# harrywaugh/UOB_Raytracer

Hardware: AMD Instinct MI355X
Metric: Mrays/sec (nominal = W*H*AA*(1+S)/t), Cornell Box 4096^2, 8xAA, 64 shadow rays (higher is better)
Workload: dtype f32; 1 GPU; headline: Cornell Box 4096x4096, 4x2 AA, 64 shadow rays, 2 spheres, <=10 bounces, 26 triangles; parallelism=1 GPU

## Files before the change

include/uob_rt.h:

```cpp
#ifndef UOB_RT_H
#define UOB_RT_H

#include <stddef.h>
#include <stdint.h>

#ifdef __cplusplus
extern "C" {
#endif

#define RT_ABI_VERSION 2
#define RT_MAX_SPHERES 4
#define RT_MAX_DEVICES 8

enum {
  RT_OK = 0,
  RT_E_INVALID = -1,
  RT_E_DEVICE = -2,
  RT_E_NOMEM = -3,
  RT_E_IO = -4,
  RT_E_UNSUPPORTED = -5
};

typedef struct rt_sphere {
  float center[3];
// ... 108 lines not shown
  float*   normal4;
  float*   albedo4;
  float*   direction4;
} rt_aov_buffers;

#define RT_AOV_ALL_SAMPLES (-1)
int rt_render_aov(rt_ctx* ctx, const float rot[12], const float cam[3], float focal, int32_t sample,
                  const rt_aov_buffers* host_out);
int rt_render_aov_device(rt_ctx* ctx, const float rot[12], const float cam[3], float focal, int32_t sample,
                         const rt_aov_buffers* device_out, void* hip_stream);
int rt_debug_aov_stats(rt_ctx* ctx, uint64_t out[8]);

int rt_debug_block_costs(rt_ctx* ctx, uint32_t* out, int32_t cap);

int rt_debug_world_masks(rt_ctx* ctx, uint64_t* out, int64_t cap, int32_t* grid, int32_t* words);

int rt_debug_tile_data(rt_ctx* ctx, int32_t* orig, float* tiles, int32_t cap_tiles);

int rt_register_output(rt_ctx* ctx, void* host, size_t bytes);
int rt_unregister_output(rt_ctx* ctx);

int rt_debug_wave_timeline(rt_ctx* ctx, uint64_t out[8]);

enum { RT_COPY_2D = 0,
       RT_COPY_PEER = 1,
       RT_COPY_LINEAR = 2    };
typedef struct rt_band_copy {
  int32_t op, reserved;
  uint64_t dst_offset, dst_pitch, src_offset, src_pitch, width_bytes, rows;
} rt_band_copy;
int rt_debug_band_copy_plan(int32_t num_devices, int32_t k, int32_t device_band_rows, int32_t width, int32_t height,
                            int32_t elem_bytes, int32_t dev_to_dev, int32_t peer_ok, int32_t same_device,
                            rt_band_copy* out, int32_t cap);

int rt_selftest_rcp(uint64_t out[64]);

int rt_selftest_normalize(uint64_t out[8], uint32_t b_stride);

void rt_destroy(rt_ctx* ctx);
const char* rt_last_error(void);
int rt_abi_version(void);

typedef struct rt_triangle {
  float v0[4], v1[4], v2[4], normal[4], color[4];
} rt_triangle;

// ... 14 lines not shown
```

uob_raytracer_amd/csrc/rt_api.hip:

```cpp
#include <cmath>
#include <cstdarg>
#include <cstdio>
#include <cstdlib>
#include <cstring>
#include <new>
#include <string>
#include <vector>

#include "rt_host.h"

namespace uobrt {

static thread_local std::string g_last_error;

void set_error(const char* fmt, ...) {
  char buf[1024];
  va_list ap;
  va_start(ap, fmt);
  vsnprintf(buf, sizeof buf, fmt, ap);
  va_end(ap);
  g_last_error = buf;
}

KeepError::KeepError() : text(g_last_error) {}
// ... 18 lines not shown
  if (!(c->light_spread >= 0.0f) || !(c->light_spread <= kMaxCoordinate)) { set_error("light_spread must be in [0, 2^16]"); return RT_E_INVALID; }
  if (validate_spheres(c->spheres, c->num_spheres) != RT_OK) return RT_E_INVALID;
  if ((double)c->width * c->height > 16777216.0) {
    set_error("width*height must not exceed 2^24 (the reference's FP32 pixel id)"); return RT_E_INVALID;
  }
  if (c->flags & 1) { set_error("flag bit 0 (the former RT_FLAG_FAST_MATH) is not defined in ABI %d", RT_ABI_VERSION); return RT_E_UNSUPPORTED; }
  if (c->num_devices < 0 || c->num_devices > RT_MAX_DEVICES || c->device_band_rows < 0) {
    set_error("num_devices must be in [0,%d] and device_band_rows >= 0", RT_MAX_DEVICES); return RT_E_INVALID;
  }
  if (c->num_devices > 1 && c->band_count != 1) {
    set_error("several devices in one context need the whole frame (band_count == 1)"); return RT_E_UNSUPPORTED;
  }
  return RT_OK;
}

static Tuning read_tuning(const rt_config& cfg) {
  Tuning t;
  if (const char* e = getenv("UOB_RT_JOB_TASKS")) t.job_tasks = atoi(e);
  if (const char* e = getenv("UOB_RT_HEAVY_FACTOR4")) { const int v = atoi(e); if (v >= 1 && v <= 4096) t.heavy_factor4 = v; }
  t.plain_order = (cfg.flags & RT_FLAG_PLAIN_ORDER) != 0 || getenv("UOB_RT_PLAIN_ORDER") != nullptr;
  t.full_grid = getenv("UOB_RT_FULL_GRID") != nullptr;
  t.no_specialise = getenv("UOB_RT_NO_SPECIALISE") != nullptr;
  if (const char* e = getenv("UOB_RT_HEAVY_DILATE")) t.heavy_dilate = atoi(e) != 0;
  if (const char* e = getenv("UOB_RT_L1_INFLATE")) { const float v = (float)atof(e); if (v >= 1.0f && v <= 64.0f) t.l1_inflate = v; }
  if (const char* e = getenv("UOB_RT_GRID_PER_CU")) { const int v = atoi(e); if (v >= 1 && v <= 8) t.grid_per_cu = v; }
  t.phase_profile = getenv("UOB_RT_PHASE_PROFILE") != nullptr;
  t.timeline = getenv("UOB_RT_TIMELINE") != nullptr;
  if (const char* e = getenv("UOB_RT_MASK_DEBUG")) t.mask_debug = atoi(e);
  if (const char* e = getenv("UOB_RT_TILE_ORDER")) t.tile_morton = !strcmp(e, "morton");
  return t;
}

extern "C" {

int rt_abi_version(void) { return RT_ABI_VERSION; }
const char* rt_last_error(void) { return g_last_error.c_str(); }

void rt_config_default(rt_config* cfg) {
  if (!cfg) return;
  memset(cfg, 0, sizeof *cfg);
  cfg->width = 1024; cfg->height = 1024;
  cfg->aa_x = 2; cfg->aa_y = 2;
  cfg->shadow_samples = 10; cfg->light_spread = 0.05f;
  cfg->max_bounces = 10;
  cfg->num_spheres = 2;
  const rt_sphere glass = {{0.3f, 0.1f, -0.5f}, 0.075f, {0.0f, 0.f, 0.f, -1.0f}};
// ... 75 lines not shown
  if (rc != RT_OK) return rc;
  if (n < 0 || (n > 0 && (!vertices4 || !normals4 || !colors4))) { set_error("scene arrays missing"); return RT_E_INVALID; }
  rc = validate_vertices(vertices4, n);
  if (rc != RT_OK) return rc;
  if (n > 4000000) { set_error("triangle list of %d exceeds the supported maximum of 4000000", n); return RT_E_UNSUPPORTED; }
  DeviceGuard guard;
  if (cfg->num_devices > 1) return init_parent(cfg, vertices4, normals4, colors4, n, out_ctx);
  int ndev = 0;
  HIP_TRY(hipGetDeviceCount(&ndev));
  if (ndev < 1) { set_error("no HIP device present"); return RT_E_DEVICE; }
  rt_ctx* c = new (std::nothrow) rt_ctx();
  if (!c) { set_error("out of host memory"); return RT_E_NOMEM; }
  c->cfg = *cfg;
  c->tune = read_tuning(*cfg);
  if (cfg->num_devices == 1) c->device = cfg->devices[0];
  else if (cfg->device >= 0) c->device = cfg->device;
  else hipGetDevice(&c->device);
  auto fail = [&](int code) { rt_destroy(c); return code; };
  if (hipSetDevice(c->device) != hipSuccess) { set_error("hipSetDevice(%d) failed", c->device); return fail(RT_E_DEVICE); }
  c->owned_rows = rt_config_owned_rows(cfg);
  if (hipDeviceGetAttribute(&c->cus, hipDeviceAttributeMultiprocessorCount, c->device) != hipSuccess || c->cus < 1) c->cus = 256;
  const size_t px = (size_t)(c->owned_rows > 0 ? c->owned_rows : 1) * cfg->width;
  if (hipMalloc(&c->d_argb, px * 4) != hipSuccess || hipMalloc(&c->d_counters, sizeof(rt_work)) != hipSuccess ||
      hipMalloc(&c->d_jobctr, (2 * kJobHeads + 2) * kJobHeadStride * sizeof(unsigned int)) != hipSuccess ||
      hipMalloc(&c->d_spheres, RT_MAX_SPHERES * sizeof(DevSphere)) != hipSuccess) {
    set_error("hipMalloc failed: %s", hipGetErrorString(hipGetLastError())); return fail(RT_E_NOMEM);
  }
  {
    const int aa = cfg->aa_x * cfg->aa_y;
    const int pt = (aa >= 1 && aa <= 64) ? 64 / aa : 16;
    const size_t jobs_max = (size_t)((cfg->width + pt - 1) / pt) * (size_t)(c->owned_rows > 0 ? c->owned_rows : 1);
    c->heavy_cap = (int)(jobs_max / 3 > 64 ? jobs_max / 3 : 64);
    c->heavy_jobs_max = jobs_max;
  }
  if (hipStreamCreate(&c->stream) != hipSuccess || hipEventCreate(&c->ev0) != hipSuccess || hipEventCreate(&c->ev1) != hipSuccess) {
    set_error("stream/event creation failed"); return fail(RT_E_DEVICE);
  }
  rc = upload_spheres(c);
  if (rc != RT_OK) return fail(rc);
  rc = scene_first(c, vertices4, normals4, colors4, n);
  if (rc != RT_OK) return fail(rc);
  *out_ctx = c;
  return RT_OK;
}

}

void uobrt::fill_params(const rt_ctx* c, const float rot[12], const float cam[3], const float light[3], float focal,
                        FrameParams* P) {
// ... 116 lines not shown
    if (!(fabsf(rot[k]) <= 4.0f)) { set_error("rotation matrix entries must be finite and <= 4"); return RT_E_INVALID; }
  if (c->owned_rows == 0) return RT_OK;
  FrameParams P;
  fill_params(c, rot, cam, light, focal, &P);
  P.out_argb = d_argb; P.out_rgb = d_rgb; P.counters = nullptr;
  P.out_global = out_global ? 1 : 0;
  HIP_TRY(hipSetDevice(c->device));
  if (c->timed && stream != c->last_stream) HIP_TRY(hipStreamWaitEvent(stream, c->ev1, 0));
  HIP_TRY(wait_aov(c, stream));
  HIP_TRY(wait_scene(c, stream));
  HIP_TRY(hipEventRecord(c->ev0, stream));
  const bool wave_paths = !(c->cfg.flags & RT_FLAG_GENERIC_KERNEL);
  if (wave_paths && wave_kernel_supports(P) && (P.aa_x * P.aa_y <= 64 || !(c->cfg.flags & RT_FLAG_NO_CULL))) {
    if (c->d_heavy_flags && P.job_tasks >= 4) {
      const int prev = c->heavy_phase, cur = prev ^ 1;
      unsigned int* const st[2] = {c->d_jobctr, c->d_jobctr + (2 * kJobHeads + 1) * kJobHeadStride};
      P.heavy_prev = c->d_heavy[prev]; P.heavy_prev_state = st[prev];
      P.heavy_new = c->d_heavy[cur]; P.heavy_new_state = st[cur];
      P.heavy_flags = c->d_heavy_flags + (size_t)prev * c->heavy_jobs_max; P.heavy_flags_new = c->d_heavy_flags + (size_t)cur * c->heavy_jobs_max;
      P.heavy_gen = ++c->heavy_gen;
      P.heavy_factor4 = c->tune.heavy_factor4;
      P.heavy_cap = P.njobs / 3 < c->heavy_cap ? P.njobs / 3 : c->heavy_cap;
      P.heavy_dilate = c->tune.heavy_dilate ? 1 : 0;
      c->heavy_phase = cur;
    }
    c->timeline_valid = false;
    if (c->tune.timeline) {
      const size_t waves = (size_t)P.wave_blocks * 4;
      if (!c->d_timeline) {
        if (hipMalloc(&c->d_timeline, waves * 3 * sizeof(uint64_t)) != hipSuccess) { set_error("hipMalloc failed (timeline)"); return RT_E_NOMEM; }
        c->timeline_waves = waves;
      }
      if (c->timeline_waves >= waves) {
        HIP_TRY(hipMemsetAsync(c->d_timeline, 0, c->timeline_waves * 3 * sizeof(uint64_t), stream));
        P.counters = reinterpret_cast<unsigned long long*>(c->d_timeline);
        c->timeline_valid = true;
      }
    }
    launch_wave(P, !(c->cfg.flags & RT_FLAG_NO_CULL), false, stream);
  } else if (wave_paths && !(c->cfg.flags & RT_FLAG_NO_CULL) && mesh_kernel_supports(P)) {
    use_tiled_scene(c, &P);
    if (c->d_mesh_cost) {
      P.mesh_order = c->mesh_order_valid ? c->d_mesh_order : nullptr;
      P.mesh_cost = c->d_mesh_cost; P.mesh_order_out = c->d_mesh_order;
      P.mesh_queue_len = c->d_mesh_order + 4 * (size_t)((c->cfg.width + 15) / 16) * (size_t)((c->owned_rows + 15) / 16);
      c->mesh_order_valid = true;
    }
    launch_stage_records(P, stream);
    launch_mesh(P, false, false, stream, c->aux_stream, c->ev_fork, c->ev_join);
  } else {
    launch_generic(P, false, stream);
  }
  HIP_TRY(hipGetLastError());
  HIP_TRY(hipEventRecord(c->ev1, stream));
  c->timed = true;
  c->last_stream = stream;
  return RT_OK;
// ... 267 lines not shown
  if (c->timed) HIP_TRY(hipStreamWaitEvent(c->stream, c->ev1, 0));
  HIP_TRY(wait_aov(c, c->stream));
  HIP_TRY(wait_scene(c, c->stream));
  HIP_TRY(hipMemsetAsync(c->d_counters, 0, sizeof(rt_work), c->stream));
  if (mesh) { use_tiled_scene(c, &P); launch_stage_records(P, c->stream); launch_mesh(P, true, c->tune.phase_profile, c->stream, nullptr, nullptr, nullptr); }
  else if (c->tune.phase_profile) launch_wave_prof(P, c->stream);
  else launch_wave(P, !(c->cfg.flags & RT_FLAG_NO_CULL), true, c->stream);
  HIP_TRY(hipGetLastError());
  HIP_TRY(hipMemcpyAsync(out, c->d_counters, sizeof(rt_work), hipMemcpyDeviceToHost, c->stream));
  HIP_TRY(hipStreamSynchronize(c->stream));
  return RT_OK;
}

int rt_debug_wave_timeline(rt_ctx* c, uint64_t out[8]) {
  if (!c || !out) { set_error("NULL argument"); return RT_E_INVALID; }
  c = lead_ctx(c);
  if (!c->tune.timeline || !c->timeline_valid) {
    set_error("rt_debug_wave_timeline: needs UOB_RT_TIMELINE=1 at rt_init and a frame rendered by the wave kernel");
    return RT_E_UNSUPPORTED;
  }
  DeviceGuard guard;
  HIP_TRY(hipSetDevice(c->device));
  if (c->timed) HIP_TRY(hipEventSynchronize(c->ev1));
  std::vector<uint64_t> rec(c->timeline_waves * 3);
  HIP_TRY(hipMemcpy(rec.data(), c->d_timeline, rec.size() * sizeof(uint64_t), hipMemcpyDeviceToHost));
  for (int q = 0; q < 8; ++q) out[q] = 0;
  out[1] = ~0ull;
  for (size_t w = 0; w < c->timeline_waves; ++w) {
    const uint64_t t0 = rec[3 * w], t1 = rec[3 * w + 1], jobs = rec[3 * w + 2] & 0xffffffffull;
    if (t1 == 0) continue;
    out[7] = rec[3 * w + 2] >> 32;
    out[0] += 1; out[3] += t0; out[4] += t1; out[5] += jobs;
    if (t0 < out[1]) out[1] = t0;
    if (t1 > out[2]) out[2] = t1;
    if (jobs > out[6]) out[6] = jobs;
  }
  return RT_OK;
}

int rt_debug_trace_rays(rt_ctx* c, int32_t what, const float* rays6, const float* radius_sq, int64_t nray,
                        int32_t* out_tri, float* out10) {
  if (!c || !rays6 || !out_tri || nray < 0) { set_error("NULL argument"); return RT_E_INVALID; }
  if (what != RT_TRACE_IN_SHADOW && what != RT_TRACE_CLOSEST_HIT) { set_error("rt_debug_trace_rays: unknown mode %d", what); return RT_E_INVALID; }
  if (what == RT_TRACE_IN_SHADOW && !radius_sq) { set_error("rt_debug_trace_rays: radius_sq missing"); return RT_E_INVALID; }
  if (what == RT_TRACE_CLOSEST_HIT && !out10) { set_error("rt_debug_trace_rays: out10 missing"); return RT_E_INVALID; }
  c = lead_ctx(c);
  if (nray == 0) return RT_OK;
  DeviceGuard guard;
  HIP_TRY(hipSetDevice(c->device));
  const float zero3[3] = {0.f, 0.f, 0.f};
  FrameParams P;
  scene_params(c, zero3, false, &P);
  float *d_rays = nullptr, *d_r2 = nullptr, *d_out = nullptr;
  int* d_tri = nullptr;
  int rc = RT_OK;
  if (hipMalloc(&d_rays, (size_t)nray * 24) != hipSuccess || hipMalloc(&d_tri, (size_t)nray * 4) != hipSuccess ||
      (radius_sq && hipMalloc(&d_r2, (size_t)nray * 4) != hipSuccess) || (out10 && hipMalloc(&d_out, (size_t)nray * 40) != hipSuccess)) {
    set_error("hipMalloc failed: %s", hipGetErrorString(hipGetLastError())); rc = RT_E_NOMEM;
// ... 128 lines not shown
```

uob_raytracer_amd/csrc/rt_device.h:

```cpp
#pragma once
#include <hip/hip_runtime.h>
#include <stdint.h>

#include "../../include/uob_rt.h"

namespace uobrt {

constexpr int kJobHeads = 31;
constexpr int kJobHeadStride = 32;
constexpr int kHeavyStateWords = 8;
constexpr float kMaxCoordinate = 65536.0f;
constexpr int kRecordsPerTriangle = 8;

struct DevSphere {
  float cx, cy, cz, r2;
  float col[4];
};

struct FrameParams {
  float rot[12];
  float cam[3];
  float focal;
  float light[3];
  float spread;
  int32_t W, H, aa_x, aa_y;
  int32_t S;
  int32_t bounces;
  int32_t nsph;
  int32_t n;
  int32_t band_rows, band_index, band_count, owned_rows;
  float sy;
  float half_wx, half_hy;
  float w_f;
// ... 13 lines not shown
  const float4* colors;
  uint32_t* out_argb;
  float4* out_rgb;
  int32_t out_global;
  int32_t wave_blocks;
  unsigned long long* counters;
  unsigned int* job_counter;
  int32_t njobs, nseg;
  int32_t aa_magic;
  int32_t aax_magic;
  int32_t job_tasks;
  int32_t no_specialise;
  const unsigned int* heavy_prev;
  const unsigned int* heavy_prev_state;
  unsigned int* heavy_new;
  unsigned int* heavy_new_state;
  const unsigned int* heavy_flags;
  unsigned int* heavy_flags_new;
  uint32_t heavy_gen;
  int32_t heavy_factor4;
  int32_t heavy_cap;
  float l1_inflate;
  int32_t heavy_dilate;
  float4* records;
  const unsigned int* mesh_order;
  unsigned int* mesh_cost;
  unsigned int* mesh_order_out;
  unsigned int* mesh_queue_len;
  int32_t mesh_blocks;
  const int* orig;
  const float4* tile_box;
  unsigned long long* screen_masks;
  unsigned long long* world_masks;
  unsigned int* world_occ;
  int32_t mask_debug;
  int32_t nwords, scx, scy, grid_g;
  float grid_lo[3], grid_cell, grid_inv;
};

struct AovPlanes {
  int* prim;
  float* depth;
  float4 *position, *normal, *albedo, *direction;
};

__device__ inline uint32_t div_magic(uint32_t n, uint32_t magic) { return magic ? __umulhi(n, magic) : n; }
// ... 13 lines not shown
```

uob_raytracer_amd/csrc/rt_host.h:

```cpp
#pragma once
#include <hip/hip_runtime.h>

#include <string>
#include <vector>

#include "rt_device.h"

#define HIP_TRY(expr)                                                                   \
  do {                                                                                  \
    hipError_t e_ = (expr);                                                             \
    if (e_ != hipSuccess) {                                                             \
      uobrt::set_error("%s failed: %s (%s:%d)", #expr, hipGetErrorString(e_), __FILE__, __LINE__); \
      return RT_E_DEVICE;                                                               \
    }                                                                                   \
  } while (0)

namespace uobrt {

void set_error(const char* fmt, ...);

struct KeepError {
  std::string text;
  KeepError();
  ~KeepError();
// ... 37 lines not shown
                     int* d_prim, float4* d_records, unsigned long long* stats, int cus, hipStream_t stream);
int aov_stats_words();
void launch_aov(const FrameParams& P, bool tiled, const AovPlanes& A, int sample, unsigned long long* stats, int cus, hipStream_t stream);
void vertex_box(const float* vertices4, int n, float lo[3], float hi[3]);
std::vector<int> tiled_order(const float* v4, int n, bool morton);
std::vector<float> tile_data_host(const float* v4, const int* orig, int n);

inline uint32_t div_magic_for(int d) { return d > 1 ? (uint32_t)((0x100000000ull + (uint64_t)d - 1) / (uint64_t)d) : 0u; }

inline int blocks_per_cu(const void* kernel, int threads) {
  int per_cu = 0;
  if (hipOccupancyMaxActiveBlocksPerMultiprocessor(&per_cu, kernel, threads, 0) != hipSuccess || per_cu < 1) per_cu = 2;
  return per_cu;
}
inline unsigned grid_blocks(long want, long cap) { return (unsigned)(want < cap ? (want > 0 ? want : 1) : cap); }

struct Tuning {
  int job_tasks = 0;
  int heavy_factor4 = 8;
  bool plain_order = false;
  bool full_grid = false;
  float l1_inflate = 3.5f;
  bool heavy_dilate = true;
  bool no_specialise = false;
  int grid_per_cu = 0;
  bool phase_profile = false;
  bool timeline = false;
  int mask_debug = 0;
  bool tile_morton = false;
};

struct DevBuffer {
  char* p = nullptr;
  size_t bytes = 0;
};
int ensure_bytes(DevBuffer* b, size_t bytes);

struct SceneStore {
  float4 *verts_m = nullptr, *normals_m = nullptr, *colors_m = nullptr, *tile_box = nullptr, *records = nullptr;
  int* orig = nullptr;
  unsigned long long *screen_masks = nullptr, *world_masks = nullptr;
  unsigned int* world_occ = nullptr;
  unsigned int *heavy[2] = {nullptr, nullptr}, *heavy_flags = nullptr, *mesh_cost = nullptr, *mesh_order = nullptr;
};

struct SideCall {
// ... 102 lines not shown
```

uob_raytracer_amd/csrc/rt_kernel_wave.hip:

```cpp
#define RT_SPHERES_IN_LDS
#define RT_RNG_JUMP_IN_LDS
#include "rt_host.h"
#include "rt_wave_common.h"

#include <type_traits>

namespace uobrt {

namespace {

constexpr int kChunk = 4;

struct WaveLds {
  float4* r0;
  float4* r1;
  float2* r2;
  float4* h0;
  float4* h1;
  uint32_t* rng;
};
__host__ __device__ constexpr int wave_lds_bytes(bool cull) {
  return (cull ? 0 : 64 * (16 + 16 + 8)) + 64 * 32 + kRngPixels * kRngStride * 4;
}

// ... 261 lines not shown
  const int PT = BIGAA ? 1 : 64 / aa;
  f3 aa_run = mk(0.f, 0.f, 0.f);
  const int GP = PT < kRngPixels ? PT : kRngPixels;
  const int gp_magic = (65536 + GP - 1) / GP;
  const f3 light = mk(P.light[0], P.light[1], P.light[2]);
  const float hbox = P.hbox;
  const unsigned long long tri_lanes = ns == 64 ? ~0ull : ((1ull << ns) - 1ull);
  const int NS = SS ? SS : P.S;
  const float inv_S = SS ? ((SS & (SS - 1)) == 0 ? 1.0f / (float)(SS ? SS : 1) : 0.0f) : P.inv_S;
  const float inv_aa = (AA_X && AA_Y) ? (((AA_X * AA_Y) & (AA_X * AA_Y - 1)) == 0 ? 1.0f / (float)(AA_X * AA_Y ? AA_X * AA_Y : 1) : 0.0f) : P.inv_aa;
  const int n_pass = MULTI ? (NS + 63) >> 6 : 1;
  const unsigned long long active = NS >= 64 ? ~0ull : ((1ull << NS) - 1ull);

  const int tl = lane < ns ? lane : 0;
  TriLane T;
  if (!CULL) {
    T = tri_lane(SC.v0, SC.e1, SC.e2, SC.c, tl);
    L.r0[lane] = make_float4(T.c.x, T.c.y, T.c.z, 0.f);
  }

  RT_STAMP(prof, 0)
  Work wk, xw;
  if (COUNT) for (int q = 0; q < 8; ++q) xw.v[q] = 0;
  int head = (int)((blockIdx.x * kWavesPerBlock + wave) % kJobHeads);
  const bool lpt = !COUNT && !PROF && PC(heavy_new) != nullptr;
  unsigned int n_heavy = 0u;
  unsigned long long heavy_thr = ~0ull;
  unsigned long long* const cost_acc = reinterpret_cast<unsigned long long*>(L.rng + 256);
  if (lpt && lane == 0) { cost_acc[0] = 0ull; cost_acc[1] = 0ull; }
  if (lpt) {
    n_heavy = PC(heavy_prev_state)[0] < (unsigned int)PC(heavy_cap) ? PC(heavy_prev_state)[0] : (unsigned int)PC(heavy_cap);
    const unsigned long long psum = ((unsigned long long)PC(heavy_prev_state)[3] << 32) | PC(heavy_prev_state)[2];
    const unsigned int pjobs = PC(heavy_prev_state)[4];
    if (pjobs != 0u) heavy_thr = (unsigned long long)PC(heavy_factor4) * (psum / pjobs) / 4ull;
  }
  const bool timeline = !COUNT && !PROF && PC(counters) != nullptr;
  unsigned long long* const tls = reinterpret_cast<unsigned long long*>(L.rng + kRngStride + 256);
  if (timeline && lane == 0) { tls[0] = __builtin_amdgcn_s_memrealtime(); tls[1] = 0ull; }
  bool phase_a = n_heavy != 0u;
  const int grid_waves = (int)gridDim.x * kWavesPerBlock;
  const int per_wave = PC(job_tasks) * PT > 32 ? 8 * grid_waves : grid_waves;
  int next_job = -1, chunk_left = 0;
  unsigned int listed = 0u;
  int chunk = PC(njobs) > 2 * per_wave ? kChunk : (PC(njobs) > per_wave ? 2 : 1);
  for (;;) {
  int job = 0;
  const int jt = PC(job_tasks);
  if (phase_a) {
    if (lane == 0) job = (int)atomicAdd(PC(job_counter) + (kJobHeads + head) * kJobHeadStride, 1u);
    const unsigned int unit = (unsigned int)__builtin_amdgcn_readfirstlane(job) * kJobHeads + (unsigned int)head;
    if (unit >= n_heavy) { phase_a = false; continue; }
    job = (int)PC(heavy_prev)[unit];
    if (job < 0 || job >= PC(njobs)) continue;
  } else {
    if (chunk_left > 0) {
      job = next_job; next_job += kJobHeads; --chunk_left; listed >>= 1;
    } else {
      if (lane == 0) job = (int)atomicAdd(PC(job_counter) + head * kJobHeadStride, (unsigned int)chunk);
      job = __builtin_amdgcn_readfirstlane(job) * kJobHeads + head;
      next_job = job + kJobHeads; chunk_left = chunk - 1;
      listed = 0u;
      if (n_heavy != 0u) {
        const int jl = job + lane * kJobHeads;
        listed = (unsigned int)ballot(lane <= chunk_left && jl < PC(njobs) && PC(heavy_flags)[jl] == PC(heavy_gen));
      }
      const int left = PC(njobs) - next_job;
      chunk = left > 2 * per_wave ? kChunk : (left > per_wave ? 2 : 1);
    }
    if (job >= PC(njobs)) {
      chunk_left = 0;
      const unsigned int at = lane < kJobHeads ? __hip_atomic_load(PC(job_counter) + lane * kJobHeadStride, __ATOMIC_RELAXED, __HIP_MEMORY_SCOPE_AGENT) : 0u;
      const unsigned long long avail = ballot(lane < kJobHeads && (long long)at * kJobHeads + lane < (long long)PC(njobs));
      if (avail == 0ull) break;
      const unsigned long long above = avail & ~((2ull << head) - 1ull);
      head = __builtin_ctzll(above != 0ull ? above : avail);
      continue;
    }
    if ((listed & 1u) != 0u) continue;
  }
  RT_STAMP(prof, 7)
  if (timeline && lane == 0) tls[1] += 1ull;
  const unsigned long long job_t0 = lpt ? __builtin_amdgcn_s_memtime() : 0ull;
  const int jrow = (int)div_magic((uint32_t)job, PC(nseg_magic));
  const int mid = (PC(owned_rows) + 1) >> 1;
  const int lr = (jrow & 1) ? mid + (jrow >> 1) : mid - 1 - (jrow >> 1);
  const int JP = BIGAA ? jt / chunks : jt * PT;
  const int x0 = (job - jrow * PC(nseg)) * JP;
  const int y = band_global_row_cold(P, lr);
  f3 outc = mk(0.f, 0.f, 0.f);
  bool jk_valid = false, jk_sph = false, jk_blocked = false;
  f3 jk_D0 = mk(0.f, 0.f, 0.f);
  float jk_ed = 0.0f;
  unsigned long long jk_K = 0ull;
  unsigned long long Kp_job = n == 64 ? ~0ull : ((1ull << n) - 1ull);
  bool sph_job = P.nsph > 0;
  if (CULL) {
    const int lnJ = opaque(lane);
    const float Xlo = (float)(x0 * aa_x) - P.half_wx;
    const float Ylo = ((float)(y * aa_y) - P.half_hy) * sy;
    const f3 wc = mk(Xlo + PC(job_hx), Ylo + PC(job_hy), P.focal);
    const f3 duc = mk(P.rot[0] * wc.x + P.rot[1] * wc.y + P.rzf[0], P.rot[4] * wc.x + P.rot[5] * wc.y + P.rzf[1],
// ... 236 lines not shown
      if (chunk == chunks - 1 && lnD == kp) outc = aa_run;
    } else {
    const f3 acc = aa_sum(contrib, aa, ((AA_X && AA_Y) ? lnD / (AA_X * AA_Y ? AA_X * AA_Y : 1) : (lnD * P.aa_magic) >> 16) * aa);
      {
        const int rel = lnD - k * PT;
        const int srcl = (rel >= 0 && rel < PT) ? rel * aa : 0;
        const f3 v = mk(shfl(acc.x, srcl), shfl(acc.y, srcl), shfl(acc.z, srcl));
        if (rel >= 0 && rel < PT) outc = v;
      }
    }
    RT_STAMP(prof, 6)
  }
  const int x = x0 + lane;
  if (!COUNT && !PROF && (BIGAA ? lane < JP : lane < jt * PT) && x < P.W) {
    const f3 c = pixel_colour(outc, aa_full, inv_aa);
    const size_t o = (size_t)(PC(out_global) ? y : lr) * P.W + x;
    PC(out_argb)[o] = pack_argb(c);
    if (PC(out_rgb)) PC(out_rgb)[o] = make_float4(c.x, c.y, c.z, 1.0f);
  }
  if (lpt) {
    const unsigned long long cost = __builtin_amdgcn_s_memtime() - job_t0;
    if (lane == 0) { cost_acc[0] += cost; cost_acc[1] += (unsigned long long)jt; }
    if (cost > heavy_thr * (unsigned long long)jt && lane < (PC(heavy_dilate) ? 3 : 1)) {
      const int jn = job + (lane == 1 ? -1 : (lane == 2 ? 1 : 0));
      const int col = jn - jrow * PC(nseg);
      if (col >= 0 && col < PC(nseg)) {
        const unsigned int was = atomicMax(PC(heavy_flags_new) + jn, PC(heavy_gen) + 1u);
        if (was < PC(heavy_gen) + 1u) {
          const unsigned int at = atomicAdd(PC(heavy_new_state), 1u);
          if (at < (unsigned int)PC(heavy_cap)) PC(heavy_new)[at] = (unsigned int)jn;
          else atomicExch(PC(heavy_flags_new) + jn, was);
        }
      }
    }
  }
  }
  if (lpt && lane == 0) {
    atomicAdd(reinterpret_cast<unsigned long long*>(PC(heavy_new_state) + 2), cost_acc[0]);
    atomicAdd(PC(heavy_new_state) + 4, (unsigned int)cost_acc[1]);
  }
  if (timeline && lane == 0) {
    const unsigned long long t1 = __builtin_amdgcn_s_memrealtime(), t0 = tls[0];
    unsigned long long* const rec = PC(counters) + 3 * (size_t)(blockIdx.x * kWavesPerBlock + wave);
    rec[0] = t0; rec[1] = t1; rec[2] = tls[1] | ((unsigned long long)n_heavy << 32);
  }
  if (PROF) {
    if (lane == 0) for (int q = 0; q < 8; ++q) atomicAdd(&PC(counters)[q], prof[q]);
    return;
  }
  if (COUNT) {
    if (lane == 0) for (int q = 0; q < 8; ++q) if (xw.v[q]) atomicAdd(&PC(counters)[q], xw.v[q]);
  }
}

template __global__ void rt_draw_wave<false, false>(const FrameParams);
template __global__ void rt_draw_wave<true, false>(const FrameParams);
template __global__ void rt_draw_wave<false, true>(const FrameParams);
template __global__ void rt_draw_wave<true, true>(const FrameParams);
template __global__ void rt_draw_wave<true, false, true>(const FrameParams);
template __global__ void rt_draw_wave<true, false, false, 32>(const FrameParams);
template __global__ void rt_draw_wave<true, false, false, 0, true>(const FrameParams);
template __global__ void rt_draw_wave<true, false, false, 32, false, 4, 2, 64>(const FrameParams);
template __global__ void rt_draw_wave<true, false, false, 32, false, 2, 2, 64>(const FrameParams);
template __global__ void rt_draw_wave<true, false, false, 32, false, 2, 2, 16>(const FrameParams);
template __global__ void rt_draw_wave<true, false, false, 32, false, 2, 2, 10>(const FrameParams);
template __global__ void rt_draw_wave<false, false, false, 0, true>(const FrameParams);
template __global__ void rt_draw_wave<true, false, false, 0, false, 0, 0, 0, true>(const FrameParams);
// ... 58 lines not shown
```

uob_raytracer_amd/csrc/rt_scene.hip:

```cpp
#include <cmath>
#include <cstring>
#include <vector>

#include "rt_host.h"

using namespace uobrt;

int uobrt::validate_spheres(const rt_sphere* sph, int num) {
  for (int i = 0; i < num; ++i) {
    const rt_sphere& s = sph[i];
    for (int k = 0; k < 3; ++k)
      if (!(fabsf(s.center[k]) <= kMaxCoordinate)) { set_error("sphere %d: |centre| must be finite and <= 2^16", i); return RT_E_INVALID; }
    if (!(fabsf(s.radius_sq) <= kMaxCoordinate * kMaxCoordinate)) { set_error("sphere %d: radius_sq must be finite and <= 2^32", i); return RT_E_INVALID; }
  }
  return RT_OK;
}

int uobrt::validate_vertices(const float* vertices4, int n) {
  for (size_t k = 0; k < (size_t)n * 12; ++k) {
    if ((k & 3) != 3 && !(fabsf(vertices4[k]) <= kMaxCoordinate)) {
      set_error("vertex %zu: coordinates must be finite and |x| <= 2^16", k / 4); return RT_E_INVALID;
    }
  }
  return RT_OK;
// ... 119 lines not shown
    get(&t->tile_box, (size_t)mesh_tiles(cap) * 3 * sizeof(float4));
  };
  auto mask_set = [&](SceneStore* t, int cap) {
    const size_t nwords = (size_t)((mesh_tiles(cap) + 63) / 64), g3 = (size_t)kWorldGrid * kWorldGrid * kWorldGrid;
    get(&t->screen_masks, (size_t)mesh_screen_cells(cfg.width) * mesh_screen_cells(cfg.height) * nwords * 8);
    get(&t->world_masks, g3 * nwords * 8);
  };
  const bool grow = n > c->cap || !c->d_verts;
  const int cap = grow ? (n > 0 ? n : 1) : c->cap;
  if (grow) {
    const size_t nb = (size_t)cap * sizeof(float4);
    g->cap = cap;
    get(&g->verts, 3 * nb); get(&g->normals, nb); get(&g->colors, nb);
    if (q.records || o.records) get(&g->t.records, (size_t)cap * kRecordsPerTriangle * sizeof(float4));
    if (q.tiled || o.verts_m) tiled_set(&g->t, cap);
    if (q.masks || o.screen_masks) mask_set(&g->t, cap);
  } else {
    if (q.records && !o.records) get(&o.records, (size_t)cap * kRecordsPerTriangle * sizeof(float4));
    if (q.tiled && !o.verts_m) tiled_set(&o, cap);
    if (q.masks && !o.screen_masks) mask_set(&o, cap);
  }
  if (q.masks && !o.world_occ) get(&o.world_occ, (size_t)mesh_occ_words(kWorldGrid) * sizeof(unsigned int));
  if (q.heavy && !o.heavy_flags) {
    get(&o.heavy[0], (size_t)c->heavy_cap * 4); get(&o.heavy[1], (size_t)c->heavy_cap * 4); get(&o.heavy_flags, 2 * c->heavy_jobs_max * 4);
  }
  if (q.mesh_sched && !o.mesh_cost) {
    const size_t jobs = (size_t)((cfg.width + 15) / 16) * (size_t)((c->owned_rows + 15) / 16);
    get(&o.mesh_cost, (jobs ? jobs : 1) * 4); get(&o.mesh_order, (4 * (jobs ? jobs : 1) + 1) * 4);
  }
  if (!ok) { set_error("hipMalloc failed: %s", hipGetErrorString(hipGetLastError())); free_growth(g); return RT_E_NOMEM; }
  if (device_tiles && q.tiled) {
    const int rc = ensure_bytes(&c->tile_scratch, tile_build_scratch_bytes(cap));
    if (rc != RT_OK) { free_growth(g); return rc; }
  }
  if (q.masks && !c->aux_stream &&
      (hipStreamCreateWithFlags(&c->aux_stream, hipStreamNonBlocking) != hipSuccess ||
       hipEventCreateWithFlags(&c->ev_fork, hipEventDisableTiming) != hipSuccess ||
       hipEventCreateWithFlags(&c->ev_join, hipEventDisableTiming) != hipSuccess)) {
    set_error("stream/event creation failed"); free_growth(g); return RT_E_DEVICE;
  }
  return RT_OK;
}

static void scene_commit(rt_ctx* c, SceneGrowth* g) {
  if (!g->cap) return;
  hipSetDevice(c->device);
  SceneStore& o = c->own;
// ... 406 lines not shown
```

uob_raytracer_amd/runtime.py:

```python
import ctypes as C
import os

import numpy as np

try:
    import torch as _torch
except ImportError:
    _torch = None

from . import abi

_HERE = os.path.dirname(os.path.abspath(__file__))
LIB_PATH = os.environ.get("UOB_RT_LIB", os.path.join(_HERE, "libuob_rt.so"))

EXPORTS = (
    "rt_abi_version", "rt_last_error", "rt_config_default", "rt_config_owned_rows", "rt_init", "rt_render",
    "rt_render_device", "rt_count_work", "rt_count_executed", "rt_last_kernel_ms", "rt_destroy", "rt_scene_cornell_box",
    "rt_scene_load_obj", "rt_scene_load_obj_ex", "rt_triangle_compute_normal", "rt_scene_pack", "rt_rotation_matrix",
    "rt_selftest_rcp", "rt_selftest_normalize", "rt_debug_trace_rays", "rt_debug_block_costs", "rt_debug_world_masks", "rt_debug_wave_timeline", "rt_register_output", "rt_unregister_output",
    "rt_debug_band_copy_plan", "rt_update_scene", "rt_update_scene_device", "rt_debug_tile_data",
    "rt_trace_rays", "rt_trace_rays_device", "rt_debug_trace_stats",
    "rt_render_aov", "rt_render_aov_device", "rt_debug_aov_stats",
    "rt_shade_points", "rt_shade_points_device", "rt_debug_shade_stats",
    "rt_radiance_rays", "rt_radiance_rays_device", "rt_debug_radiance_stats",
    "rt_replace_scene", "rt_replace_scene_device", "rt_update_spheres", "rt_debug_scene_capacity",
    "rt_scene_transform", "rt_set_objects", "rt_pose_objects", "rt_pose_objects_device", "rt_debug_object_count",
)

TRACE_STATS_KEYS = ("rays", "waves", "tiles", "bundle_tiles", "tested_tiles", "triangle_tests", "unculled_rays", "reserved")
AOV_STATS_KEYS = ("samples", "waves", "tiles", "mask_tiles", "tested_tiles", "triangle_tests", "reserved6", "reserved7")

SHADE_STATS_KEYS = ("points", "sample_rays", "waves", "tiles", "bundle_tiles", "tested_tiles", "triangle_tests", "skipped_points")

RADIANCE_STATS_KEYS = ("rays", "bounce_rays", "shaded_points", "sample_rays", "closest_tested_tiles", "closest_triangle_tests",
                       "shadow_triangle_tests", "unculled_rays")

_lib = None


class RtError(RuntimeError):
    def __init__(self, code, msg):
        super().__init__("libuob_rt: error %d: %s" % (code, msg))
# ... 32 lines not shown
        L.rt_count_executed.argtypes = [vp, fp, fp, fp, C.c_float, C.POINTER(C.c_uint64)]
        L.rt_last_kernel_ms.argtypes = [vp, fp]
        L.rt_destroy.argtypes = [vp]
        L.rt_destroy.restype = None
        L.rt_scene_cornell_box.argtypes = [C.POINTER(abi.RtTriangle), C.c_int32]
        L.rt_scene_load_obj.argtypes = [C.c_char_p, C.POINTER(abi.RtTriangle), C.c_int32]
        L.rt_scene_load_obj_ex.argtypes = [C.c_char_p, fp, C.c_float, fp, C.POINTER(abi.RtTriangle), C.c_int32]
        L.rt_debug_trace_rays.argtypes = [vp, C.c_int32, fp, fp, C.c_int64, C.POINTER(C.c_int32), fp]
        L.rt_trace_rays.argtypes = [vp, C.c_int32, fp, fp, C.c_int64, C.POINTER(C.c_int32), fp]
        L.rt_trace_rays_device.argtypes = [vp, C.c_int32, vp, vp, C.c_int64, vp, vp, vp]
        L.rt_debug_trace_stats.argtypes = [vp, C.POINTER(C.c_uint64)]
        L.rt_render_aov.argtypes = [vp, fp, fp, C.c_float, C.c_int32, C.POINTER(abi.RtAovBuffers)]
        L.rt_render_aov_device.argtypes = [vp, fp, fp, C.c_float, C.c_int32, C.POINTER(abi.RtAovBuffers), vp]
        L.rt_debug_aov_stats.argtypes = [vp, C.POINTER(C.c_uint64)]
        L.rt_shade_points.argtypes = [vp, fp, C.POINTER(C.c_int32), C.c_int64, fp, fp, C.POINTER(C.c_int32)]
        L.rt_shade_points_device.argtypes = [vp, vp, vp, C.c_int64, fp, vp, vp, vp]
        L.rt_debug_shade_stats.argtypes = [vp, C.POINTER(C.c_uint64)]
        L.rt_radiance_rays.argtypes = [vp, fp, C.POINTER(C.c_int32), C.c_int64, fp, fp, C.POINTER(C.c_int32)]
        L.rt_radiance_rays_device.argtypes = [vp, vp, vp, C.c_int64, fp, vp, vp, vp]
        L.rt_debug_radiance_stats.argtypes = [vp, C.POINTER(C.c_uint64)]
        L.rt_debug_block_costs.argtypes = [vp, C.POINTER(C.c_uint32), C.c_int32]
        L.rt_debug_world_masks.argtypes = [vp, C.POINTER(C.c_uint64), C.c_int64, C.POINTER(C.c_int32), C.POINTER(C.c_int32)]
        L.rt_debug_wave_timeline.argtypes = [vp, C.POINTER(C.c_uint64)]
        L.rt_debug_band_copy_plan.argtypes = [C.c_int32] * 9 + [C.POINTER(abi.RtBandCopy), C.c_int32]
        L.rt_register_output.argtypes = [vp, vp, C.c_size_t]
        L.rt_unregister_output.argtypes = [vp]
        L.rt_triangle_compute_normal.argtypes = [C.POINTER(abi.RtTriangle)]
        L.rt_triangle_compute_normal.restype = None
        L.rt_scene_pack.argtypes = [C.POINTER(abi.RtTriangle), C.c_int32, fp, fp, fp]
        L.rt_scene_pack.restype = None
        L.rt_rotation_matrix.argtypes = [C.c_float, C.c_float, fp]
        L.rt_rotation_matrix.restype = None
        if L.rt_abi_version() != abi.RT_ABI_VERSION:
            raise ImportError("libuob_rt.so ABI %d != binding %d" % (L.rt_abi_version(), abi.RT_ABI_VERSION))
        _lib = L
    return _lib


def _check(rc):
    if rc < 0:
        raise RtError(rc, lib().rt_last_error().decode(errors="replace"))
    return rc


def _fp(a):
    return a.ctypes.data_as(C.POINTER(C.c_float))
# ... 536 lines not shown
        xs = (torch.arange(width, **f32) + 0.5) * torch.tensor(2.0 * math.pi, **f32) / torch.tensor(float(width), **f32)
        phi = torch.tensor(float(yaw), **f32) + xs - torch.tensor(math.pi, **f32)
        theta = (torch.arange(height, **f32) + 0.5) * torch.tensor(math.pi, **f32) / torch.tensor(float(height), **f32) \
            - torch.tensor(math.pi / 2.0, **f32)
        ct = torch.cos(theta)[:, None]
        d = torch.stack([torch.sin(phi)[None, :] * ct, torch.sin(theta)[:, None].expand(height, width),
                         torch.cos(phi)[None, :] * ct], -1)
        start = torch.tensor(np.ascontiguousarray(cam, np.float32)[:3].copy(), device=dev).expand(height, width, 3)
        rays = torch.cat([start, d], -1).reshape(-1, 6).contiguous()
        seeds = (torch.arange(width * height, dtype=torch.int64, device=dev) & abi.RT_SHADE_SEED_MASK).to(torch.int32)
        return self.radiance_rays_device(rays, light, seeds=seeds).reshape(height, width, 4)

    def trace_stats(self):
        return self._stats("rt_debug_trace_stats", TRACE_STATS_KEYS)

    def wave_timeline(self):
        out = (C.c_uint64 * 8)()
        _check(lib().rt_debug_wave_timeline(self._h, out))
        n = max(int(out[0]), 1)
        first, last = int(out[1]), int(out[2])
        return {"waves": int(out[0]), "span_us": (last - first) / 100.0, "mean_start_us": (int(out[3]) / n - first) / 100.0,
                "mean_idle_tail_us": (last - int(out[4]) / n) / 100.0, "jobs": int(out[5]), "max_jobs_per_wave": int(out[6]), "listed_jobs": int(out[7])}

    def world_masks(self):
        g, w = C.c_int32(), C.c_int32()
        n = _check(lib().rt_debug_world_masks(self._h, None, 0, C.byref(g), C.byref(w)))
        out = np.zeros(n, np.uint64)
        _check(lib().rt_debug_world_masks(self._h, out.ctypes.data_as(C.POINTER(C.c_uint64)), n, C.byref(g), C.byref(w)))
        return out.reshape(g.value, g.value, g.value, w.value)

    def block_costs(self):
        n = _check(lib().rt_debug_block_costs(self._h, None, 0))
        out = np.zeros(n, np.uint32)
        _check(lib().rt_debug_block_costs(self._h, out.ctypes.data_as(C.POINTER(C.c_uint32)), n))
        return out.reshape((self.rows + 15) // 16, (self.width + 15) // 16)

    def last_kernel_ms(self):
        ms = C.c_float()
        _check(lib().rt_last_kernel_ms(self._h, C.byref(ms)))
        return float(ms.value)
```

Measured before the change: 3.954 million Mrays/s.

## Add cost classes to heavy-job list and per-SIMD split of list vs plain waves

```diff
diff --git a/include/uob_rt.h b/include/uob_rt.h
--- a/include/uob_rt.h
+++ b/include/uob_rt.h
@@ -154,6 +154,8 @@
 
 int rt_debug_wave_timeline(rt_ctx* ctx, uint64_t out[8]);
 
+int rt_debug_wave_phases(rt_ctx* ctx, uint64_t out[16]);
+
 enum { RT_COPY_2D = 0,
        RT_COPY_PEER = 1,
        RT_COPY_LINEAR = 2    };
diff --git a/uob_raytracer_amd/csrc/rt_api.hip b/uob_raytracer_amd/csrc/rt_api.hip
--- a/uob_raytracer_amd/csrc/rt_api.hip
+++ b/uob_raytracer_amd/csrc/rt_api.hip
@@ -64,6 +64,9 @@
   t.full_grid = getenv("UOB_RT_FULL_GRID") != nullptr;
   t.no_specialise = getenv("UOB_RT_NO_SPECIALISE") != nullptr;
   if (const char* e = getenv("UOB_RT_HEAVY_DILATE")) t.heavy_dilate = atoi(e) != 0;
+  if (const char* e = getenv("UOB_RT_LIST_WGS")) { const int v = atoi(e); if (v >= 0 && v <= 8) t.list_wgs = v; }
+  if (const char* e = getenv("UOB_RT_HEAVY_CLASSES")) { const int v = atoi(e); if (v >= 1 && v <= kHeavyClasses) t.heavy_classes = v; }
+  if (const char* e = getenv("UOB_RT_HEAVY_CLASS_SHIFT")) { const int v = atoi(e); if (v >= 1 && v <= 4) t.heavy_class_shift = v; }
   if (const char* e = getenv("UOB_RT_L1_INFLATE")) { const float v = (float)atof(e); if (v >= 1.0f && v <= 64.0f) t.l1_inflate = v; }
   if (const char* e = getenv("UOB_RT_GRID_PER_CU")) { const int v = atoi(e); if (v >= 1 && v <= 8) t.grid_per_cu = v; }
   t.phase_profile = getenv("UOB_RT_PHASE_PROFILE") != nullptr;
@@ -185,9 +188,12 @@
   if (hipDeviceGetAttribute(&c->cus, hipDeviceAttributeMultiprocessorCount, c->device) != hipSuccess || c->cus < 1) c->cus = 256;
   const size_t px = (size_t)(c->owned_rows > 0 ? c->owned_rows : 1) * cfg->width;
   if (hipMalloc(&c->d_argb, px * 4) != hipSuccess || hipMalloc(&c->d_counters, sizeof(rt_work)) != hipSuccess ||
-      hipMalloc(&c->d_jobctr, (2 * kJobHeads + 2) * kJobHeadStride * sizeof(unsigned int)) != hipSuccess ||
+      hipMalloc(&c->d_jobctr, ((2 * kJobHeads + 2) * kJobHeadStride + kSimdSlotWords) * sizeof(unsigned int)) != hipSuccess ||
       hipMalloc(&c->d_spheres, RT_MAX_SPHERES * sizeof(DevSphere)) != hipSuccess) {
     set_error("hipMalloc failed: %s", hipGetErrorString(hipGetLastError())); return fail(RT_E_NOMEM);
+  }
+  if (hipMemset(c->d_jobctr + (2 * kJobHeads + 2) * kJobHeadStride, 0, kSimdSlotWords * sizeof(unsigned int)) != hipSuccess) {
+    set_error("hipMemset failed: %s", hipGetErrorString(hipGetLastError())); return fail(RT_E_DEVICE);
   }
   {
     const int aa = cfg->aa_x * cfg->aa_y;
@@ -350,17 +356,22 @@
       P.heavy_factor4 = c->tune.heavy_factor4;
       P.heavy_cap = P.njobs / 3 < c->heavy_cap ? P.njobs / 3 : c->heavy_cap;
       P.heavy_dilate = c->tune.heavy_dilate ? 1 : 0;
+      P.heavy_stride = c->heavy_cap;
+      P.heavy_classes = c->tune.heavy_classes; P.heavy_class_shift = c->tune.heavy_class_shift;
+      P.simd_waves = P.wave_blocks / c->cus > 0 ? P.wave_blocks / c->cus : 1;
+      P.list_waves = c->tune.list_wgs < 0 || c->tune.list_wgs > P.simd_waves ? P.simd_waves : c->tune.list_wgs;
+      if (P.list_waves < P.simd_waves && P.heavy_classes > 1) P.simd_slots = c->d_jobctr + (2 * kJobHeads + 2) * kJobHeadStride;
       c->heavy_phase = cur;
     }
     c->timeline_valid = false;
     if (c->tune.timeline) {
       const size_t waves = (size_t)P.wave_blocks * 4;
       if (!c->d_timeline) {
-        if (hipMalloc(&c->d_timeline, waves * 3 * sizeof(uint64_t)) != hipSuccess) { set_error("hipMalloc failed (timeline)"); return RT_E_NOMEM; }
+        if (hipMalloc(&c->d_timeline, waves * kTimelineWords * sizeof(uint64_t)) != hipSuccess) { set_error("hipMalloc failed (timeline)"); return RT_E_NOMEM; }
         c->timeline_waves = waves;
       }
       if (c->timeline_waves >= waves) {
-        HIP_TRY(hipMemsetAsync(c->d_timeline, 0, c->timeline_waves * 3 * sizeof(uint64_t), stream));
+        HIP_TRY(hipMemsetAsync(c->d_timeline, 0, c->timeline_waves * kTimelineWords * sizeof(uint64_t), stream));
         P.counters = reinterpret_cast<unsigned long long*>(c->d_timeline);
         c->timeline_valid = true;
       }
@@ -674,18 +685,59 @@
   DeviceGuard guard;
   HIP_TRY(hipSetDevice(c->device));
   if (c->timed) HIP_TRY(hipEventSynchronize(c->ev1));
-  std::vector<uint64_t> rec(c->timeline_waves * 3);
+  std::vector<uint64_t> rec(c->timeline_waves * kTimelineWords);
   HIP_TRY(hipMemcpy(rec.data(), c->d_timeline, rec.size() * sizeof(uint64_t), hipMemcpyDeviceToHost));
   for (int q = 0; q < 8; ++q) out[q] = 0;
   out[1] = ~0ull;
   for (size_t w = 0; w < c->timeline_waves; ++w) {
-    const uint64_t t0 = rec[3 * w], t1 = rec[3 * w + 1], jobs = rec[3 * w + 2] & 0xffffffffull;
+    const uint64_t t0 = rec[kTimelineWords * w], t1 = rec[kTimelineWords * w + 1], jobs = rec[kTimelineWords * w + 2] & 0xffffffffull;
     if (t1 == 0) continue;
-    out[7] = rec[3 * w + 2] >> 32;
+    out[7] = rec[kTimelineWords * w + 2] >> 32;
     out[0] += 1; out[3] += t0; out[4] += t1; out[5] += jobs;
     if (t0 < out[1]) out[1] = t0;
     if (t1 > out[2]) out[2] = t1;
     if (jobs > out[6]) out[6] = jobs;
+  }
+  return RT_OK;
+}
+
+int rt_debug_wave_phases(rt_ctx* c, uint64_t out[16]) {
+  if (!c || !out) { set_error("NULL argument"); return RT_E_INVALID; }
+  c = lead_ctx(c);
+  if (!c->tune.timeline || !c->timeline_valid) {
+    set_error("rt_debug_wave_phases: needs UOB_RT_TIMELINE=1 at rt_init and a frame rendered by the wave kernel");
+    return RT_E_UNSUPPORTED;
+  }
+  DeviceGuard guard;
+  HIP_TRY(hipSetDevice(c->device));
+  if (c->timed) HIP_TRY(hipEventSynchronize(c->ev1));
+  std::vector<uint64_t> rec(c->timeline_waves * kTimelineWords);
+  HIP_TRY(hipMemcpy(rec.data(), c->d_timeline, rec.size() * sizeof(uint64_t), hipMemcpyDeviceToHost));
+  for (int q = 0; q < 16; ++q) out[q] = 0;
+  uint64_t first = ~0ull;
+  for (size_t w = 0; w < c->timeline_waves; ++w)
+    if (rec[kTimelineWords * w + 1] != 0 && rec[kTimelineWords * w] < first) first = rec[kTimelineWords * w];
+  std::vector<uint8_t> roles(kSimdSlotWords, 0);
+  for (size_t w = 0; w < c->timeline_waves; ++w) {
+    const uint64_t* r = &rec[kTimelineWords * w];
+    if (r[1] == 0) continue;
+    const uint64_t listed = r[4] & 0xffffffffull, simd = (r[4] >> 32) & (kSimdSlotWords - 1), plain = (r[4] >> 48) & 1;
+    if (r[3] != 0) {
+      const uint64_t d = r[3] - first;
+      out[0] += 1; out[1] += d;
+      if (d > out[2]) out[2] = d;
+    }
+    out[3] += listed;
+    if (listed > out[4]) out[4] = listed;
+    if (plain) { out[7] += 1; out[8] += listed; }
+    if ((r[2] >> 32) != 0) roles[simd] |= plain ? 2 : 1;
+  }
+  for (int s = 0; s < kSimdSlotWords; ++s) { out[5] += roles[s] != 0; out[6] += roles[s] == 3; }
+  if (c->d_heavy_flags) {
+    unsigned int st[kHeavyStateWords];
+    const unsigned int* const d_st = (c->heavy_phase ^ 1) ? c->d_jobctr + (2 * kJobHeads + 1) * kJobHeadStride : c->d_jobctr;
+    HIP_TRY(hipMemcpy(st, d_st, sizeof st, hipMemcpyDeviceToHost));
+    for (int k = 0; k < kHeavyClasses; ++k) out[9 + k] = st[kHeavyClassWord + k];
   }
   return RT_OK;
 }
diff --git a/uob_raytracer_amd/csrc/rt_device.h b/uob_raytracer_amd/csrc/rt_device.h
--- a/uob_raytracer_amd/csrc/rt_device.h
+++ b/uob_raytracer_amd/csrc/rt_device.h
@@ -8,7 +8,11 @@
 
 constexpr int kJobHeads = 31;
 constexpr int kJobHeadStride = 32;
-constexpr int kHeavyStateWords = 8;
+constexpr int kHeavyStateWords = 12;
+constexpr int kHeavyClasses = 4;
+constexpr int kHeavyClassWord = 8;
+constexpr int kSimdSlotWords = 1 << 14;
+constexpr int kTimelineWords = 5;
 constexpr float kMaxCoordinate = 65536.0f;
 constexpr int kRecordsPerTriangle = 8;
 
@@ -68,6 +72,11 @@
   int32_t heavy_cap;
   float l1_inflate;
   int32_t heavy_dilate;
+  int32_t heavy_stride;
+  int32_t heavy_classes;
+  int32_t heavy_class_shift;
+  int32_t list_waves, simd_waves;
+  unsigned int* simd_slots;
   float4* records;
   const unsigned int* mesh_order;
   unsigned int* mesh_cost;
diff --git a/uob_raytracer_amd/csrc/rt_host.h b/uob_raytracer_amd/csrc/rt_host.h
--- a/uob_raytracer_amd/csrc/rt_host.h
+++ b/uob_raytracer_amd/csrc/rt_host.h
@@ -83,6 +83,9 @@
   bool full_grid = false;
   float l1_inflate = 3.5f;
   bool heavy_dilate = true;
+  int list_wgs = -1;
+  int heavy_classes = 1;
+  int heavy_class_shift = 1;
   bool no_specialise = false;
   int grid_per_cu = 0;
   bool phase_profile = false;
diff --git a/uob_raytracer_amd/csrc/rt_kernel_wave.hip b/uob_raytracer_amd/csrc/rt_kernel_wave.hip
--- a/uob_raytracer_amd/csrc/rt_kernel_wave.hip
+++ b/uob_raytracer_amd/csrc/rt_kernel_wave.hip
@@ -307,22 +307,38 @@
   RT_STAMP(prof, 0)
   Work wk, xw;
   if (COUNT) for (int q = 0; q < 8; ++q) xw.v[q] = 0;
-  int head = (int)((blockIdx.x * kWavesPerBlock + wave) % kJobHeads);
+  constexpr int kInList = 1 << 16;
+  constexpr int kSeenPlain = 1 << 17;
+  constexpr int kTopOnly = 1 << 18;
+  int sched = (int)((blockIdx.x * kWavesPerBlock + wave) % kJobHeads) * 0x101;
   const bool lpt = !COUNT && !PROF && PC(heavy_new) != nullptr;
   unsigned int n_heavy = 0u;
   unsigned long long heavy_thr = ~0ull;
   unsigned long long* const cost_acc = reinterpret_cast<unsigned long long*>(L.rng + 256);
   if (lpt && lane == 0) { cost_acc[0] = 0ull; cost_acc[1] = 0ull; }
   if (lpt) {
-    n_heavy = PC(heavy_prev_state)[0] < (unsigned int)PC(heavy_cap) ? PC(heavy_prev_state)[0] : (unsigned int)PC(heavy_cap);
+    for (int c = 0; c < kHeavyClasses; ++c) n_heavy += PC(heavy_prev_state)[kHeavyClassWord + c];
+    if (n_heavy > (unsigned int)PC(heavy_cap)) n_heavy = (unsigned int)PC(heavy_cap);
     const unsigned long long psum = ((unsigned long long)PC(heavy_prev_state)[3] << 32) | PC(heavy_prev_state)[2];
     const unsigned int pjobs = PC(heavy_prev_state)[4];
     if (pjobs != 0u) heavy_thr = (unsigned long long)PC(heavy_factor4) * (psum / pjobs) / 4ull;
   }
   const bool timeline = !COUNT && !PROF && PC(counters) != nullptr;
   unsigned long long* const tls = reinterpret_cast<unsigned long long*>(L.rng + kRngStride + 256);
-  if (timeline && lane == 0) { tls[0] = __builtin_amdgcn_s_memrealtime(); tls[1] = 0ull; }
-  bool phase_a = n_heavy != 0u;
+  unsigned long long* const tlp = reinterpret_cast<unsigned long long*>(L.rng + 2 * kRngStride + 256);
+  if (timeline && lane == 0) { tls[0] = __builtin_amdgcn_s_memrealtime(); tls[1] = 0ull; tlp[0] = 0ull; tlp[1] = 0ull; }
+  sched |= n_heavy != 0u ? kInList : kSeenPlain;
+  if (lpt && n_heavy != 0u && (timeline || PC(simd_slots) != nullptr)) {
+    const unsigned int hw = __builtin_amdgcn_s_getreg((31 << 11) | 4), xcc = __builtin_amdgcn_s_getreg((3 << 11) | 20);
+    const unsigned int simd = ((xcc & 15u) << 10) | (((hw >> 8) & 255u) << 2) | ((hw >> 4) & 3u);
+    if (PC(simd_slots) != nullptr) {
+      unsigned int slot = 0u;
+      if (lane == 0) slot = atomicAdd(PC(simd_slots) + simd, 1u);
+      slot = (unsigned int)__builtin_amdgcn_readfirstlane((int)slot);
+      if (slot % (unsigned int)PC(simd_waves) >= (unsigned int)PC(list_waves)) sched |= kTopOnly;
+    }
+    if (timeline && lane == 0) tlp[1] = ((unsigned long long)simd << 32) | ((sched & kTopOnly) ? 1ull << 48 : 0ull);
+  }
   const int grid_waves = (int)gridDim.x * kWavesPerBlock;
   const int per_wave = PC(job_tasks) * PT > 32 ? 8 * grid_waves : grid_waves;
   int next_job = -1, chunk_left = 0;
@@ -331,13 +347,36 @@
   for (;;) {
   int job = 0;
   const int jt = PC(job_tasks);
-  if (phase_a) {
-    if (lane == 0) job = (int)atomicAdd(PC(job_counter) + (kJobHeads + head) * kJobHeadStride, 1u);
-    const unsigned int unit = (unsigned int)__builtin_amdgcn_readfirstlane(job) * kJobHeads + (unsigned int)head;
-    if (unit >= n_heavy) { phase_a = false; continue; }
-    job = (int)PC(heavy_prev)[unit];
-    if (job < 0 || job >= PC(njobs)) continue;
+  bool dry = false;
+  if ((sched & kInList) != 0) {
+    const int lh = (sched >> 8) & 31;
+    if (lane == 0) job = (int)atomicAdd(PC(job_counter) + (kJobHeads + lh) * kJobHeadStride, 1u);
+    const unsigned int unit = (unsigned int)__builtin_amdgcn_readfirstlane(job) * kJobHeads + (unsigned int)lh;
+    if (unit >= n_heavy) {
+      if ((sched & kSeenPlain) == 0) {
+        sched = (sched & ~(kInList | kTopOnly)) | kSeenPlain;
+        if (timeline && lane == 0 && tlp[0] == 0ull) tlp[0] = __builtin_amdgcn_s_memrealtime();
+        continue;
+      }
+      dry = true;
+    } else {
+      int c = PC(heavy_classes) - 1;
+      if ((sched & kTopOnly) != 0 && unit >= PC(heavy_prev_state)[kHeavyClassWord + c]) {
+        sched = (sched & ~(kInList | kTopOnly)) | kSeenPlain;
+        if (timeline && lane == 0 && tlp[0] == 0ull) tlp[0] = __builtin_amdgcn_s_memrealtime();
+      }
+      unsigned int u = unit;
+      for (; c > 0; --c) {
+        const unsigned int cnt = PC(heavy_prev_state)[kHeavyClassWord + c];
+        if (u < cnt) break;
+        u -= cnt;
+      }
+      job = u < (unsigned int)PC(heavy_stride) ? (int)PC(heavy_prev)[(size_t)c * (size_t)PC(heavy_stride) + u] : -1;
+      if (job < 0 || job >= PC(njobs)) continue;
+      if (timeline && lane == 0) tlp[1] += 1ull;
+    }
   } else {
+    const int head = sched & 31;
     if (chunk_left > 0) {
       job = next_job; next_job += kJobHeads; --chunk_left; listed >>= 1;
     } else {
@@ -352,16 +391,24 @@
       const int left = PC(njobs) - next_job;
       chunk = left > 2 * per_wave ? kChunk : (left > per_wave ? 2 : 1);
     }
-    if (job >= PC(njobs)) {
-      chunk_left = 0;
-      const unsigned int at = lane < kJobHeads ? __hip_atomic_load(PC(job_counter) + lane * kJobHeadStride, __ATOMIC_RELAXED, __HIP_MEMORY_SCOPE_AGENT) : 0u;
-      const unsigned long long avail = ballot(lane < kJobHeads && (long long)at * kJobHeads + lane < (long long)PC(njobs));
-      if (avail == 0ull) break;
-      const unsigned long long above = avail & ~((2ull << head) - 1ull);
-      head = __builtin_ctzll(above != 0ull ? above : avail);
-      continue;
-    }
-    if ((listed & 1u) != 0u) continue;
+    if (job >= PC(njobs)) { chunk_left = 0; dry = true; }
+    else if ((listed & 1u) != 0u) continue;
+  }
+  if (dry) {
+    const int hq = lane & 31;
+    const bool lst = lane >= 32;
+    const unsigned int at = hq < kJobHeads ? __hip_atomic_load(PC(job_counter) + ((lst ? kJobHeads : 0) + hq) * kJobHeadStride, __ATOMIC_RELAXED, __HIP_MEMORY_SCOPE_AGENT) : 0u;
+    const unsigned long long avail = ballot(hq < kJobHeads && (long long)at * kJobHeads + hq < (lst ? (long long)n_heavy : (long long)PC(njobs)));
+    if (avail == 0ull) break;
+    const unsigned int av_plain = (unsigned int)avail, av_list = (unsigned int)(avail >> 32);
+    if (av_plain != 0u) {
+      const unsigned int above = av_plain & ~((2u << (sched & 31)) - 1u);
+      sched = (sched & ~(31 | kInList)) | __builtin_ctz(above != 0u ? above : av_plain) | kSeenPlain;
+    } else {
+      const unsigned int above = av_list & ~((2u << ((sched >> 8) & 31)) - 1u);
+      sched = (sched & ~(31 << 8)) | (__builtin_ctz(above != 0u ? above : av_list) << 8) | kInList;
+    }
+    continue;
   }
   RT_STAMP(prof, 7)
   if (timeline && lane == 0) tls[1] += 1ull;
@@ -644,13 +691,18 @@
     const unsigned long long cost = __builtin_amdgcn_s_memtime() - job_t0;
     if (lane == 0) { cost_acc[0] += cost; cost_acc[1] += (unsigned long long)jt; }
     if (cost > heavy_thr * (unsigned long long)jt && lane < (PC(heavy_dilate) ? 3 : 1)) {
+      int cls = 0;
+      for (int b = 1; b < PC(heavy_classes); ++b) cls += cost > ((heavy_thr * (unsigned long long)jt) << (b * PC(heavy_class_shift))) ? 1 : 0;
       const int jn = job + (lane == 1 ? -1 : (lane == 2 ? 1 : 0));
       const int col = jn - jrow * PC(nseg);
       if (col >= 0 && col < PC(nseg)) {
         const unsigned int was = atomicMax(PC(heavy_flags_new) + jn, PC(heavy_gen) + 1u);
         if (was < PC(heavy_gen) + 1u) {
           const unsigned int at = atomicAdd(PC(heavy_new_state), 1u);
-          if (at < (unsigned int)PC(heavy_cap)) PC(heavy_new)[at] = (unsigned int)jn;
+          if (at < (unsigned int)PC(heavy_cap)) {
+            const unsigned int pos = atomicAdd(PC(heavy_new_state) + kHeavyClassWord + cls, 1u);
+            PC(heavy_new)[(size_t)cls * (size_t)PC(heavy_stride) + pos] = (unsigned int)jn;
+          }
           else atomicExch(PC(heavy_flags_new) + jn, was);
         }
       }
@@ -663,8 +715,9 @@
   }
   if (timeline && lane == 0) {
     const unsigned long long t1 = __builtin_amdgcn_s_memrealtime(), t0 = tls[0];
-    unsigned long long* const rec = PC(counters) + 3 * (size_t)(blockIdx.x * kWavesPerBlock + wave);
+    unsigned long long* const rec = PC(counters) + kTimelineWords * (size_t)(blockIdx.x * kWavesPerBlock + wave);
     rec[0] = t0; rec[1] = t1; rec[2] = tls[1] | ((unsigned long long)n_heavy << 32);
+    rec[3] = tlp[0]; rec[4] = tlp[1];
   }
   if (PROF) {
     if (lane == 0) for (int q = 0; q < 8; ++q) atomicAdd(&PC(counters)[q], prof[q]);
diff --git a/uob_raytracer_amd/csrc/rt_scene.hip b/uob_raytracer_amd/csrc/rt_scene.hip
--- a/uob_raytracer_amd/csrc/rt_scene.hip
+++ b/uob_raytracer_amd/csrc/rt_scene.hip
@@ -165,7 +165,8 @@
   }
   if (q.masks && !o.world_occ) get(&o.world_occ, (size_t)mesh_occ_words(kWorldGrid) * sizeof(unsigned int));
   if (q.heavy && !o.heavy_flags) {
-    get(&o.heavy[0], (size_t)c->heavy_cap * 4); get(&o.heavy[1], (size_t)c->heavy_cap * 4); get(&o.heavy_flags, 2 * c->heavy_jobs_max * 4);
+    get(&o.heavy[0], (size_t)c->heavy_cap * kHeavyClasses * 4); get(&o.heavy[1], (size_t)c->heavy_cap * kHeavyClasses * 4);
+    get(&o.heavy_flags, 2 * c->heavy_jobs_max * 4);
   }
   if (q.mesh_sched && !o.mesh_cost) {
     const size_t jobs = (size_t)((cfg.width + 15) / 16) * (size_t)((c->owned_rows + 15) / 16);
diff --git a/uob_raytracer_amd/runtime.py b/uob_raytracer_amd/runtime.py
--- a/uob_raytracer_amd/runtime.py
+++ b/uob_raytracer_amd/runtime.py
@@ -17,7 +17,7 @@
     "rt_abi_version", "rt_last_error", "rt_config_default", "rt_config_owned_rows", "rt_init", "rt_render",
     "rt_render_device", "rt_count_work", "rt_count_executed", "rt_last_kernel_ms", "rt_destroy", "rt_scene_cornell_box",
     "rt_scene_load_obj", "rt_scene_load_obj_ex", "rt_triangle_compute_normal", "rt_scene_pack", "rt_rotation_matrix",
-    "rt_selftest_rcp", "rt_selftest_normalize", "rt_debug_trace_rays", "rt_debug_block_costs", "rt_debug_world_masks", "rt_debug_wave_timeline", "rt_register_output", "rt_unregister_output",
+    "rt_selftest_rcp", "rt_selftest_normalize", "rt_debug_trace_rays", "rt_debug_block_costs", "rt_debug_world_masks", "rt_debug_wave_timeline", "rt_debug_wave_phases", "rt_register_output", "rt_unregister_output",
     "rt_debug_band_copy_plan", "rt_update_scene", "rt_update_scene_device", "rt_debug_tile_data",
     "rt_trace_rays", "rt_trace_rays_device", "rt_debug_trace_stats",
     "rt_render_aov", "rt_render_aov_device", "rt_debug_aov_stats",
@@ -96,6 +96,8 @@
         L.rt_debug_block_costs.argtypes = [vp, C.POINTER(C.c_uint32), C.c_int32]
         L.rt_debug_world_masks.argtypes = [vp, C.POINTER(C.c_uint64), C.c_int64, C.POINTER(C.c_int32), C.POINTER(C.c_int32)]
         L.rt_debug_wave_timeline.argtypes = [vp, C.POINTER(C.c_uint64)]
+        if hasattr(L, "rt_debug_wave_phases"):
+            L.rt_debug_wave_phases.argtypes = [vp, C.POINTER(C.c_uint64)]
         L.rt_debug_band_copy_plan.argtypes = [C.c_int32] * 9 + [C.POINTER(abi.RtBandCopy), C.c_int32]
         L.rt_register_output.argtypes = [vp, vp, C.c_size_t]
         L.rt_unregister_output.argtypes = [vp]
@@ -678,6 +680,14 @@
         return {"waves": int(out[0]), "span_us": (last - first) / 100.0, "mean_start_us": (int(out[3]) / n - first) / 100.0,
                 "mean_idle_tail_us": (last - int(out[4]) / n) / 100.0, "jobs": int(out[5]), "max_jobs_per_wave": int(out[6]), "listed_jobs": int(out[7])}
 
+    def wave_phases(self):
+        out = (C.c_uint64 * 16)()
+        _check(lib().rt_debug_wave_phases(self._h, out))
+        n = max(int(out[0]), 1)
+        return {"waves_left_list": int(out[0]), "mean_list_phase_us": int(out[1]) / n / 100.0, "last_list_phase_us": int(out[2]) / 100.0,
+                "listed_jobs_run": int(out[3]), "max_listed_jobs_per_wave": int(out[4]), "simds": int(out[5]), "simds_with_both_roles": int(out[6]),
+                "plain_waves": int(out[7]), "listed_jobs_run_by_plain_waves": int(out[8]), "class_entries": [int(out[9 + k]) for k in range(4)]}
+
     def world_masks(self):
         g, w = C.c_int32(), C.c_int32()
         n = _check(lib().rt_debug_world_masks(self._h, None, 0, C.byref(g), C.byref(w)))
```

Result: no change. 3.917 million Mrays/s (-0.9%).
